# andres-fr/realtime-pose-estimation

Hardware: AMD Instinct MI355X
Metric: images/sec at 640x640 (HRNet-w48 fwd+decode) (higher is better)
Workload: dtype f16 (fp32 accumulate, fp32 BatchNorm; fp32 NCHW in/out); 1 GPU; configs[2]: batch=32 per GPU, 640x640, half-wrapper teacher forward + decode of 17 keypoint channels, weights W0 (seeded random); batch_per_gpu=32, people_per_batch_rank0=960

## Files before the change

### realtime-pose-estimation_amd/csrc/engine.hip

```cpp
#include <stdarg.h>

#include <chrono>
#include <mutex>
#include <map>
#include <tuple>
#include <vector>

#include "rtpe_common.h"

namespace rtpe {

static thread_local std::string g_err;

void set_error(const char* fmt, ...) {
  char buf[1024];
  va_list ap;
  va_start(ap, fmt);
  vsnprintf(buf, sizeof(buf), fmt, ap);
  va_end(ap);
  g_err = buf;
}

int hip_fail(hipError_t e, const char* what, const char* file, int line) {
  set_error("HIP error %d (%s) at %s:%d: %s", (int)e, hipGetErrorString(e), file, line, what);
// ... 9 lines not shown
  int n_geom;
  int fuse;
  int pair;
  int proj_head;
  int proj_op;
  int stem2;
  int s2g;
};

}

using namespace rtpe;

enum {
  kRouteNone = 0,
  kRouteTile, kRouteStream, kRouteDirect, kRouteConv64,
  kRouteHead,
  kRouteS2,
  kRouteS2Group,
  kRouteDeconvMerged, kRouteDeconv48,
  kRoutePairHead, kRoutePairTail, kRoutePairProj,
  kRouteBlock,
  kRouteStemFused, kRouteStemConv1, kRouteStemPlain,
  kRouteDoneBy
};
static_assert(kRouteTile == RTPE_ROUTE_TILE && kRouteHead == RTPE_ROUTE_HEAD && kRouteS2 == RTPE_ROUTE_S2 && kRouteS2Group == RTPE_ROUTE_S2_GROUP &&
              kRouteDeconvMerged == RTPE_ROUTE_DECONV_MERGED && kRoutePairHead == RTPE_ROUTE_PAIR_HEAD && kRoutePairTail == RTPE_ROUTE_PAIR_TAIL &&
              kRoutePairProj == RTPE_ROUTE_PAIR_PROJ && kRouteBlock == RTPE_ROUTE_BLOCK && kRouteStemFused == RTPE_ROUTE_STEM_FUSED &&
              kRouteStemConv1 == RTPE_ROUTE_STEM_CONV1 && kRouteStemPlain == RTPE_ROUTE_STEM_PLAIN && kRouteDoneBy == RTPE_ROUTE_DONE_BY,
              "rtpe_hip_trace.h names other route numbers");

static void trace_put(std::vector<int32_t>* tr, int kind, int a, int b, int c = 0, int d = 0) {
  const int32_t r[RTPE_TRACE_INTS] = {kind, a, b, c, d};
  tr->insert(tr->end(), r, r + RTPE_TRACE_INTS);
}

struct Route {
  int how, by;
  ConvTile tile[4];
};

struct rtpe_record {
  std::vector<hipEvent_t> ev;
  std::vector<Route> routes;
};

struct rtpe_hrnet {
// ... 1 lines not shown
  std::vector<OpState> ops;
  std::map<std::tuple<int, int, int>, std::vector<ConvTile>> tuned;
  std::map<int, rtpe_record> records;
  std::vector<rtpe_tensor_desc> tensors;
  std::vector<char> plane_ok;
  int n_slots;
  char* arena;
  size_t arena_bytes;
  int n_preds, n_refined;
  std::mutex lane_mu;
  hipStream_t lane_stream[4] = {nullptr, nullptr, nullptr, nullptr};
  std::vector<hipEvent_t> op_event;
  std::vector<char> needs_event;
  std::vector<std::vector<int>> wait_ops;
  hipEvent_t fork_event = nullptr;
  bool has_regions = false;
  std::vector<int32_t> trace;
  bool any_size = false;
};

static size_t align_up(size_t v, size_t a) { return (v + a - 1) / a * a; }

namespace rtpe {
static int g_options[kNumOptions] = {-1, -1, -1, -1, -1, -1, -1, -1, -1, -1, -1, -1};
static const char* const kOptionNames[kNumOptions] = {"block_ring", "block_pc", "direct_1x1", "lanes", "tile_dma", "pair_1x1", "fused_stem", "conv64", "head_direct", "deconv48", "conv48s2", "pair_proj"};
static const char* const kOptionEnv[kNumOptions] = {"RTPE_BLOCK_RING", "RTPE_BLOCK_PC", "RTPE_DIRECT_1X1", "RTPE_LANES", "RTPE_TILE_DMA", "RTPE_PAIR_1X1", "RTPE_FUSED_STEM", "RTPE_CONV64", "RTPE_HEAD_DIRECT", "RTPE_DECONV48", "RTPE_CONV48S2", "RTPE_PAIR_PROJ"};
static const int kOptionDefault[kNumOptions] = {0, 1, 1, 1, 1, 1, 1, 1, 1, 1, 1, 1};
int get_option(int key) {
  int v = __atomic_load_n(&g_options[key], __ATOMIC_RELAXED);
  if (v < 0) {
    v = kOptionEnv[key][0] ? env_int(kOptionEnv[key], kOptionDefault[key]) : kOptionDefault[key];
    __atomic_store_n(&g_options[key], v, __ATOMIC_RELAXED);
  }
  return v;
}
}

extern "C" int rtpe_set_option(const char* name, int32_t value) {
  RTPE_REQUIRE(name != nullptr && value >= 0, "set_option: bad argument");
  for (int k = 0; k < kNumOptions; ++k)
    if (kOptionNames[k][0] && strcmp(name, kOptionNames[k]) == 0) {
      __atomic_store_n(&g_options[k], (int)value, __ATOMIC_RELAXED);
      return RTPE_OK;
    }
  set_error("set_option: unknown option '%s'", name);
  return RTPE_E_INVALID;
}

extern "C" int rtpe_get_option(const char* name, int32_t* value) {
  RTPE_REQUIRE(name != nullptr && value != nullptr, "get_option: null argument");
  for (int k = 0; k < kNumOptions; ++k)
    if (kOptionNames[k][0] && strcmp(name, kOptionNames[k]) == 0) {
      *value = get_option(k);
      return RTPE_OK;
// ... 425 lines not shown

static std::vector<char> plane_tensors(const rtpe_hrnet* h, int N, int H, int W, const std::vector<ConvTile>* tuned, bool rag) {
  if (rag) return std::vector<char>(h->plane_ok.size(), 0);
  std::vector<char> plane = h->plane_ok;
  for (size_t i = 0; i < h->ops.size(); ++i) {
    const OpState& o = h->ops[i];
    const rtpe_op_desc& d = o.d;
    if (d.kind != RTPE_OP_CONV || o.n_geom != 1) continue;
    if (!(plane[d.in_t] || plane[d.out_t] || (d.res_t >= 0 && plane[d.res_t]))) continue;
    const rtpe_tensor_desc& ti = h->tensors[d.in_t];
    const ConvTile t = (tuned && (*tuned)[i * 4].nt) ? (*tuned)[i * 4]
                                                      : conv_make_tile(o.plan[0], N, extent(H, ti.ds_log2), extent(W, ti.ds_log2));
    if (t.kind != 2) {
      plane[d.in_t] = plane[d.out_t] = 0;
      if (d.res_t >= 0) plane[d.res_t] = 0;
    }
  }
  return plane;
}

struct RouteOpts {
  int fused_stem = get_option(kOptFusedStem), pair_1x1 = get_option(kOptPair1x1), pair_proj = get_option(kOptPairProj),
      conv64 = get_option(kOptConv64), head_direct = get_option(kOptHeadDirect), deconv48 = get_option(kOptDeconv48),
      conv48s2 = get_option(kOptConv48s2);
};

struct Fwd {
  const rtpe_hrnet* h;
  int N, H, W;
  char* base;
  void *preds, *refined;
  int out_dtype;
  std::vector<size_t> offs;
  size_t ws_need;
  const std::vector<ConvTile>* tuned = nullptr;
  std::vector<char> plane;
  bool rag;
  const int32_t* ext;
  const int32_t* level(int ds) const { return ext + (size_t)ds * 2 * N; }
  Fwd(const rtpe_hrnet* h_, int N_, int H_, int W_, void* ws, void* preds_, void* refined_, int out_dtype_, const int32_t* ext_ = nullptr)
      : h(h_), N(N_), H(H_), W(W_), base(reinterpret_cast<char*>(ws)), preds(preds_), refined(refined_), out_dtype(out_dtype_),
        rag(ragged(H_, W_) || ext_ != nullptr), ext(ext_) {
    slot_layout(h, N, H, W, &offs, &ws_need);
    auto it = h->tuned.find(std::make_tuple(N, H, W));
    if (it != h->tuned.end() && !rag) tuned = &it->second;
    plane = plane_tensors(h, N, H, W, tuned, rag);
  }
// ... 72 lines not shown
    a.ext_in = f.level(ti.ds_log2);
    a.ext_out = f.level(ti.ds_log2 + (d.stride == 2 ? 1 : 0));
  }
  return a;
}

static ConvArgs conv_op_args(const Fwd& f, size_t i, int k, const ConvTile& t) {
  ConvArgs a = conv_op_args(f, i, k);
  conv_fill_args(f.h->ops[i].geom[k], f.h->ops[i].plan[k], t, &a);
  return a;
}

static bool conv_direct_ok(const ConvArgs& a) {
  return a.x_bytes < 0x80000000ull && a.y != nullptr && a.y_nchw == nullptr && a.o_mul == 1;
}

static void conv_fix_tile(const RouteOpts& opt, const ConvPlan& p, const ConvArgs& a, bool plane_io, ConvTile* t) {
  const bool direct_ok = conv_direct_ok(a);
  if (t->kind == 4 && !direct_ok) *t = conv_make_tile(p, a.N, a.H_pos, a.W_pos, false);
  if (t->kind == 5 && !(direct_ok && a.res == nullptr && !plane_io && opt.conv64 != 0))
    *t = conv_make_tile(p, a.N, a.H_pos, a.W_pos, true, false);
}

static int conv_pick(const RouteOpts& opt, const ConvPlan& p, const ConvTile& t, const ConvArgs& a, bool plane_io) {
  if (opt.head_direct != 0 && conv_head_supports(p, a)) return kRouteHead;
  if (opt.conv48s2 != 0 && !plane_io && conv48s2_supports(p, a)) return kRouteS2;
  return t.kind == 2 ? kRouteStream : t.kind == 4 ? kRouteDirect : t.kind == 5 ? kRouteConv64 : kRouteTile;
}

static bool deconv_merges(const ConvPlan* p, const ConvTile& tile0) {
  static const int merge_deconv = env_int("RTPE_DECONV_MERGE", 1);
  bool merge = merge_deconv && tile0.kind == 0;
  for (int k = 1; k < 4 && merge; ++k)
    merge = p[k].mt == p[0].mt && p[k].cc == p[0].cc && p[k].kc == p[0].kc && p[k].n_cchunks == p[0].n_cchunks &&
            p[k].n_cb == p[0].n_cb && p[k].pstride == p[0].pstride && p[k].tapw == p[0].tapw;
  return merge;
}

static void deconv_merge_class(ConvArgs* merged, const ConvArgs& a, int k) {
  if (k == 0) { *merged = a; merged->n_cls = 4; }
  merged->w_c[k] = a.w;
  merged->lo_yc[k] = a.lo_y; merged->lo_xc[k] = a.lo_x;
  merged->oy_c[k] = a.oy_add; merged->ox_c[k] = a.ox_add;
}

static ConvArgs deconv_merged_args(const Fwd& f, size_t i, const ConvTile& tile0) {
  ConvArgs merged;
  for (int k = 0; k < 4; ++k) deconv_merge_class(&merged, conv_op_args(f, i, k, tile0), k);
  return merged;
}

static int deconv_pick(const RouteOpts& opt, const ConvPlan& p0, const ConvArgs& merged) {
  return opt.deconv48 != 0 && deconv48_supports(p0, merged) ? kRouteDeconv48 : kRouteDeconvMerged;
}

static int launch_conv(int how, const ConvPlan& p, const ConvTile& t, const ConvArgs& a, hipStream_t s) {
  switch (how) {
    case kRouteHead: return conv_head_launch(p, a, s);
    case kRouteS2: return conv48s2_launch(p, a, s);
    case kRouteDeconv48: return deconv48_launch(p, a, s);
    default: return conv_launch(p, t, a, s);
  }
}

static int route_ops(const Fwd& f, std::vector<Route>* routes, std::vector<ConvArgs>* args) {
  const rtpe_hrnet* h = f.h;
  const RouteOpts opt;
  routes->assign(h->ops.size(), Route());
  args->assign(h->ops.size(), ConvArgs());
  for (size_t i = 0; i < h->ops.size(); ++i) {
    Route& r = (*routes)[i];
    const OpState& o = h->ops[i];
    const rtpe_op_desc& d = o.d;
    auto absorb = [&](size_t j) { (*routes)[j].how = kRouteDoneBy; (*routes)[j].by = (int)i; };
    if (r.how == kRouteDoneBy) continue;
    if (d.kind == RTPE_OP_STEM) {
      const int fused = !f.rag && stem_fused_supports(f.H, f.W) ? opt.fused_stem : 0;
      r.how = fused == 1 && o.stem2 == 1 ? kRouteStemFused : fused == 2 && !(d.flags & RTPE_F_F32) ? kRouteStemConv1 : kRouteStemPlain;
      if (r.how == kRouteStemFused) absorb(i + 1);
      continue;
    }
    if (o.n_geom == 0) continue;
// ... 21 lines not shown
    if (o.s2g > 1 && opt.conv48s2 != 0) {
      bool ok = true;
      for (int m = 0; m < o.s2g && ok; ++m) {
        const OpState& om = h->ops[i + m];
        Route& rm = (*routes)[i + m];
        if (m > 0) rm.tile[0] = f.tile(i + m, 0, Hi / 2, Wi / 2);
        (*args)[i + m] = conv_op_args(f, i + m, 0, rm.tile[0]);
        ok = !f.plane[om.d.in_t] && !f.plane[om.d.out_t] && conv48s2_supports(om.plan[0], (*args)[i + m]);
      }
      if (ok) {
        r.how = kRouteS2Group;
        r.by = o.s2g;
        for (int m = 1; m < o.s2g; ++m) absorb(i + m);
        continue;
      }
    }
    const bool plane_io = f.plane[d.in_t] || (!(d.flags & RTPE_F_NO_NHWC) && f.plane[d.out_t]);
    ConvArgs& a = (*args)[i];
    a = conv_op_args(f, i, 0);
    for (int k = 0; k < o.n_geom; ++k) conv_fix_tile(opt, o.plan[k], k ? conv_op_args(f, i, k) : a, plane_io, &r.tile[k]);
    conv_fill_args(o.geom[0], o.plan[0], r.tile[0], &a);
    if (r.how == kRoutePairTail) continue;
    r.how = conv_pick(opt, o.plan[0], r.tile[0], a, plane_io);
    if (r.how == kRouteHead || r.how == kRouteS2 || opt.pair_1x1 == 0 || !conv_direct_ok(a)) continue;
    if (o.proj_head > 0 && opt.pair_proj != 0 && conv_direct_ok(conv_op_args(f, o.proj_head, 0))) {
      r.how = kRoutePairProj;
      r.by = o.proj_head + 1;
    } else if (o.pair == 1) {
      r.how = kRoutePairHead;
      r.by = (int)i + 1;
      (*routes)[i + 1].how = kRoutePairTail;
      (*routes)[i + 1].by = (int)i;
    }
  }
  for (size_t i = 0; i < h->ops.size(); ++i)
    RTPE_REQUIRE((*routes)[i].how != kRoutePairProj || (*routes)[h->ops[i].proj_head].how == kRoutePairHead,
                 "forward: op %d is no 1x1 pair head at this shape, its projection was folded", h->ops[i].proj_head);
  return RTPE_OK;
}

static void route_label(const rtpe_hrnet* h, const std::vector<Route>& routes, size_t i, int32_t* out8) {
  const Route& r = routes[i];
  const OpState& o = h->ops[i];
  const ConvTile& t = r.tile[0];
  const int by = r.how == kRouteDoneBy ? routes[r.by].how : kRouteNone;
  auto set = [&](int mt, int nt, int waves, int th, int tw, int cc, int n_cb, int v) {
    const int32_t l[8] = {mt, nt, waves, th, tw, cc, n_cb, v};
    memcpy(out8, l, sizeof(l));
  };
  memset(out8, 0, 8 * sizeof(int32_t));
  if (r.how == kRouteStemFused || by == kRouteStemFused) {
    set(4, 4, 8, 8, 16, 64, 1, by ? -600002 : -600001);
  } else if (r.how == kRouteBlock || by == kRouteBlock) {
    set(3, by ? 3 : 5, 4, 6, 32, 48, 1, by ? -900002 : -900001);
  } else if (r.how == kRouteS2 || r.how == kRouteS2Group || by == kRouteS2Group) {
    const int gw = o.d.cout == 48 ? 1 : o.d.cout == 96 ? 2 : 4;
    set(3, 2, 4, 8, 8, 48, o.d.cout / (48 * gw), by ? -200009 : r.how == kRouteS2Group ? -(200000 + r.by) : -200001);
  } else if (r.how == kRouteHead) {
    set(o.plan[0].mt, 2, 4, 1, 32, 48, 1, -400001);
  } else if (r.how == kRouteDeconv48) {
    set(3, 2, 4, 8, 16, 48, 1, -300001);
  } else if (r.how == kRoutePairProj) {
    set(0, 1, 8, 1, 16, 64, 1, -800003);
  } else if (r.how == kRoutePairHead || r.how == kRoutePairTail) {
    const bool head = r.how == kRoutePairHead;
    set(head ? 16 : 4, 1, 8, 1, 16, head ? 64 : 256, 1, head ? -800001 : -800002);
  } else if (o.n_geom > 0) {
    set(t.kind == 0 && t.mrun ? t.mrun : o.plan[0].mt, t.nt, t.waves, t.th, t.tw, o.plan[0].cc, o.plan[0].n_cb,
        t.kind == 2 ? -(t.grid + 100000 * t.n_bufs) : t.kind == 4 ? -(700000 + t.grid) : t.kind == 5 ? -(500000 + t.grid) : (int32_t)t.lds_bytes);
  }
}

static bool block_head(const std::vector<Route>& r, size_t i) { return i < r.size() && r[i].how == kRouteBlock; }
static bool block_tail(const std::vector<Route>& r, size_t i) { return i > 0 && block_head(r, i - 1); }

static bool op_has_event(const std::vector<Route>& r, size_t i) {
  return !block_tail(r, i) && !(block_head(r, i) && block_head(r, i + 2));
}

static int read_op_times(const std::vector<Route>& r, const std::vector<hipEvent_t>& ev, float* op_ms) {
// ... 219 lines not shown
  const Route& r = routes[i];
  switch (r.how) {
    case kRouteDoneBy: case kRoutePairHead: case kRoutePairProj:
      return RTPE_OK;
    case kRouteStemFused: case kRouteStemConv1:
      return stem_fused_launch(stem_fused_args(f, c, i, r.how == kRouteStemFused), s);
    case kRouteStemPlain:
      return stem_launch(stem_args(f, c, i), s);
    case kRouteBlock:
      return launch_block(f, i, s);
    case kRouteS2Group: {
      const ConvPlan* plans[3];
      for (int m = 0; m < r.by; ++m) plans[m] = &h->ops[i + m].plan[0];
      return conv48s2_launch_group(plans, &args[i], r.by, s);
    }
    case kRoutePairTail: {
      const OpState& oh = h->ops[r.by];
      const bool proj = oh.proj_op >= 0 && routes[oh.proj_op].how == kRoutePairProj;
      return conv_pair_launch(oh.plan[0], args[r.by], o.plan[0], args[i], s, proj ? &h->ops[oh.proj_op].plan[0] : nullptr,
                              proj ? &args[oh.proj_op] : nullptr);
    }
    case kRouteDeconvMerged: case kRouteDeconv48:
      return launch_conv(r.how, o.plan[0], r.tile[0], args[i], s);
    case kRouteTile: case kRouteStream: case kRouteDirect: case kRouteConv64: case kRouteHead: case kRouteS2: {
      int rc = launch_conv(r.how, o.plan[0], r.tile[0], args[i], s);
      for (int k = 1; k < o.n_geom && rc == RTPE_OK; ++k)
        rc = launch_conv(r.how, o.plan[k], r.tile[k], conv_op_args(f, i, k, r.tile[k]), s);
      return rc;
    }
    default:
      break;
  }
  switch (o.d.kind) {
    case RTPE_OP_CAST: case RTPE_OP_AUX_PACK: case RTPE_OP_RESIZE: case RTPE_OP_GATE_MUL:
      return launch_f32_op(f, c, i, s);
    case RTPE_OP_AVGPOOL: case RTPE_OP_SE: case RTPE_OP_CAM_COMBINE: case RTPE_OP_SIGMOID_ADD:
      return (o.d.flags & RTPE_F_F32) ? launch_student_op<float>(f, c, i, s) : launch_student_op<_Float16>(f, c, i, s);
    default:
      return launch_fuse(f, i, s);
  }
}

class Lanes {
 public:
  Lanes(rtpe_hrnet* h, const FwdCall& c, const std::vector<Route>& routes, std::vector<int32_t>* trace)
      : h_(h), routes_(routes), main_(c.stream), tr_(trace) {
    if (h->has_regions && c.op_ms == nullptr && c.rec == nullptr && !(c.flags & RTPE_FWD_NO_LANES)) {
// ... 434 lines not shown
  a.alpha = reinterpret_cast<const float*>(dev + wb); a.beta = a.alpha + p.cout_pad;
  a.res = reinterpret_cast<const _Float16*>(res); a.res_ld = cout;
  a.y = reinterpret_cast<_Float16*>(y); a.out_ld = cout; a.cout_store = cout;
  a.N = N; a.H_in = H; a.W_in = W;
  a.H_full = a.H_pos = H / stride; a.W_full = a.W_pos = W / stride; a.o_mul = 1;
  a.relu = (flags & RTPE_F_RELU) ? 1 : 0;
  a.round_conv = (flags & RTPE_F_ROUND_CONV) ? 1 : 0;
  const RouteOpts opt;
  ConvTile tile = conv_make_tile(p, N, a.H_pos, a.W_pos);
  conv_fix_tile(opt, p, a, false, &tile);
  static const int probe_plane = RTPE_DIAG_ENV_INT("RTPE_PROBE_PLANE", 0);
  if (probe_plane && tile.kind == 2 && cin % 48 == 0 && cout % 48 == 0 && stride == 1) {
    a.in_ld = 48; a.in_cs = (long long)N * H * W * 48;
    a.out_ld = 48; a.out_cs = (long long)N * H * W * 48;
    if (res != nullptr) { a.res_ld = 48; a.res_cs = (long long)N * H * W * 48; }
  }
  conv_fill_args(g, p, tile, &a);
#ifdef RTPE_CONV_STAMPS
  unsigned long long* dbg = nullptr;
  hipMalloc(reinterpret_cast<void**>(&dbg), 128);
  hipMemset(dbg, 0, 128);
  a.dbg = dbg;
#endif
  int rc = launch_conv(conv_pick(opt, p, tile, a, false), p, tile, a, s);
  hipError_t es2 = hipStreamSynchronize(s);
#ifdef RTPE_CONV_STAMPS
  unsigned long long hd[16];
  hipMemcpy(hd, dbg, 128, hipMemcpyDeviceToHost);
  hipFree(dbg);
  if (tile.kind == 2 && hd[5] && (hd[11] = hd[11] ? hd[11] : hd[5] / tile.waves)) {
    const unsigned long long nw = (unsigned long long)tile.grid * tile.waves, units = hd[5] / p.n_cchunks;
    fprintf(stderr, "stream conv %dx%d nt%d w%d nb%d nw%d grid %d | per MFMA wave: total %llu cycles, %llu units | per stage: waitM %llu half0 %llu "
            "waitH %llu half1 %llu | per unit: E-wait %llu bn+transpose %llu res-wait %llu rows+add+store %llu load_res %llu | weight loader/stage: wait %llu issue %llu | "
            "tile loaders/stage: wait %llu issue %llu\n",
            tile.th, tile.tw, tile.nt, tile.waves, tile.n_bufs, tile.n_wslots, tile.grid, hd[15] / nw, units / nw, hd[0] / hd[5], hd[1] / hd[5],
            hd[2] / hd[5], hd[3] / hd[5], hd[12] / units, hd[13] / units, hd[4] / units, hd[14] / units, hd[10] / units, hd[6] / hd[11],
            hd[7] / hd[11], hd[8] / hd[11], hd[9] / hd[11]);
  }
  else if (hd[5])
    fprintf(stderr, "conv stamps (kind %d): n %llu | per wave(-unit) cycles: setup %llu stage/wait1 %llu kloop %llu epilogue %llu total/wait2 %llu\n",
            tile.kind, hd[5], hd[0] / hd[5], hd[1] / hd[5], hd[2] / hd[5], hd[3] / hd[5], hd[4] / hd[5]);
  if (hd[10] && tile.kind != 2)
    fprintf(stderr, "   loader per stage: vmcnt-wait %llu barrier1 %llu issue %llu barriersE+2 %llu (stages %llu)\n",
            hd[6] / hd[10], hd[7] / hd[10], hd[8] / hd[10], hd[9] / hd[10], hd[10]);
#endif
  hipFree(dev);
  if (rc != RTPE_OK) return rc;
  if (es2 != hipSuccess) return hip_fail(es2, "hipStreamSynchronize", __FILE__, __LINE__);
  return RTPE_OK;
}

extern "C" int rtpe_basicblock_nhwc(const void* x, int32_t N, int32_t H, int32_t W, const void* w1_host,
                                    const float* alpha1, const float* beta1, const void* w2_host, const float* alpha2,
                                    const float* beta2, void* y, void* stream) {
  RTPE_REQUIRE(x && w1_host && w2_host && alpha1 && beta1 && alpha2 && beta2 && y, "basicblock_nhwc: null argument");
  RTPE_REQUIRE(conv_block_supports(48, 48, H, W), "basicblock_nhwc: H=%d W=%d unsupported", H, W);
  hipStream_t s = reinterpret_cast<hipStream_t>(stream);
  ConvGeom g{48, 48, 3, 1, -1, 2, 1};
  ConvPlan p = conv_make_plan(g);
  const size_t wb = align_up(p.packed_bytes, 256), abb = align_up(2 * 48 * sizeof(float), 256);
// ... 346 lines not shown
```

### realtime-pose-estimation_amd/csrc/rtpe_common.h

```cpp
#pragma once
#include <hip/hip_runtime.h>
#include <hip/hip_fp16.h>
#include <stdint.h>
#include <stdio.h>
#include <stdlib.h>
#include <string.h>
#include <string>
#include <vector>

#include "rtpe_hip.h"

namespace rtpe {

void set_error(const char* fmt, ...);
int hip_fail(hipError_t e, const char* what, const char* file, int line);

#define RTPE_HIP_CHECK(expr)                                               \
  do {                                                                     \
    hipError_t _e = (expr);                                                \
    if (_e != hipSuccess) return ::rtpe::hip_fail(_e, #expr, __FILE__, __LINE__); \
  } while (0)

#define RTPE_REQUIRE(cond, ...)                 \
  do {                                          \
    if (!(cond)) {                              \
      ::rtpe::set_error(__VA_ARGS__);           \
      return RTPE_E_INVALID;                    \
    }                                           \
  } while (0)

inline int env_int(const char* name, int dflt) {
  const char* v = getenv(name);
  return v ? atoi(v) : dflt;
}
#ifdef RTPE_DIAG
#define RTPE_DIAG_ENV_INT(name, dflt) ::rtpe::env_int(name, dflt)
#else
#define RTPE_DIAG_ENV_INT(name, dflt) (dflt)
#endif

enum { kOptBlockRing = 0, kOptBlockPC = 1, kOptDirect1x1 = 2, kOptLanes = 3, kOptTileDma = 4, kOptPair1x1 = 5, kOptFusedStem = 6, kOptConv64 = 7, kOptHeadDirect = 8, kOptDeconv48 = 9, kOptConv48s2 = 10, kOptPairProj = 11, kNumOptions = 12 };
int get_option(int key);

inline bool first_use_on_device(unsigned long long* mask) {
  int dev = 0;
  if (hipGetDevice(&dev) != hipSuccess || dev < 0 || dev > 63) return true;
  const unsigned long long bit = 1ull << dev;
  const unsigned long long old = __atomic_fetch_or(mask, bit, __ATOMIC_RELAXED);
  return !(old & bit);
}

struct DeviceGuard {
  int prev = -1;
  bool switched = false;
  hipError_t err = hipSuccess;
  explicit DeviceGuard(int device) {
    err = hipGetDevice(&prev);
    if (err == hipSuccess && prev != device) {
      err = hipSetDevice(device);
      switched = err == hipSuccess;
    }
  }
  ~DeviceGuard() {
    if (switched) (void)hipSetDevice(prev);
// ... 132 lines not shown
void conv_enum_tiles(const ConvPlan& p, int N, int H_pos, int W_pos, std::vector<ConvTile>* out);
void conv_pack_weights(const ConvGeom& g, const ConvPlan& p, const void* w, void* packed);
void conv_fill_args(const ConvGeom& g, const ConvPlan& p, const ConvTile& t, ConvArgs* a);
int conv_launch(const ConvPlan& p, const ConvTile& t, const ConvArgs& a, hipStream_t s);
bool conv_stream_supports(const ConvPlan& p);
size_t conv_stream_lds(const ConvPlan& p, int buf_bytes, int n_bufs, int n_wslots);
int conv_stream_launch(const ConvPlan& p, const ConvTile& t, const ConvArgs& a, hipStream_t s);
bool conv_pair_supports(int cin1, int cout1, int cout2);
int conv_pair_launch(const ConvPlan& p1, const ConvArgs& c1, const ConvPlan& p2, const ConvArgs& c2, hipStream_t s,
                     const ConvPlan* pd = nullptr, const ConvArgs* cd = nullptr);
int conv_direct_mb(const ConvPlan& p);
bool conv64_supports(const ConvPlan& p);
size_t conv64_lds();
int conv64_grid(int N, int H_pos, int W_pos);
int conv64_launch(const ConvPlan& p, const ConvTile& t, const ConvArgs& a, hipStream_t s);
int conv_direct_launch(const ConvPlan& p, const ConvArgs& a, hipStream_t s);
bool conv_head_supports(const ConvPlan& p, const ConvArgs& a);
int conv_head_launch(const ConvPlan& p, const ConvArgs& a, hipStream_t s);
bool deconv48_supports(const ConvPlan& p, const ConvArgs& merged);
int deconv48_launch(const ConvPlan& p, const ConvArgs& merged, hipStream_t s);
bool conv48s2_supports(const ConvPlan& p, const ConvArgs& a);
int conv48s2_launch(const ConvPlan& p, const ConvArgs& a, hipStream_t s);
int conv48s2_launch_group(const ConvPlan* const* plans, const ConvArgs* layers, int n, hipStream_t s);
bool conv_block_supports(int cin, int cout, int H, int W);
int conv_block_launch(const _Float16* x, int in_ld, size_t x_bytes, _Float16* y, int out_ld, const _Float16* w1,
                      const float* ab1, const _Float16* w2, const float* ab2, int N, int H, int W, hipStream_t s);

struct FuseArgs {
  const _Float16* term[4];
  int term_ld[4], term_up[4];
  int n_terms;
  _Float16* y;
  int out_ld, C;
  int N, H, W;
  int f32;
  int relu;
  int nearest;
  int term_h[4], term_w[4];
  const int* ext_out;
  const int* ext_term[4];
};
int fuse_launch(const FuseArgs& a, hipStream_t s);
bool fuse_nearest_supports(int N, int H, int W, int C, int f32);

struct StemArgs {
  const void* x;
// ... 54 lines not shown
```

Baseline: 2480 images/sec.

## Add warp-specialized stride-2 3x3 conv kernel for wide-channel transition layers

Adds a new stride-2 3x3 convolution kernel with dedicated loader waves. One wave streams weights and two waves stream input tiles into LDS through double-buffered buffer-to-LDS loads, while four MFMA waves compute and run a fused BN/ReLU epilogue. It is routed by default for the 96->192/384 and 192->384 downsampling layers and replaces the generic stream or tile conv path for them. It adds another specialized kernel and more barrier synchronization in exchange for better overlap of memory and compute on these layers.

```diff
diff --git a/include/rtpe_hip_s2c.h b/include/rtpe_hip_s2c.h
--- /dev/null
+++ b/include/rtpe_hip_s2c.h
@@ -0,0 +1,20 @@
+#ifndef RTPE_HIP_S2C_H
+#define RTPE_HIP_S2C_H
+
+#include <stdint.h>
+
+#ifdef __cplusplus
+extern "C" {
+#endif
+
+int rtpe_conv_s2c_probe(int32_t cin, int32_t cout, int32_t ksize, int32_t stride, int32_t N, int32_t H, int32_t W,
+                        int32_t in_ld, int32_t plane, int32_t with_res, int32_t small_grid, int32_t* out10);
+
+int rtpe_conv_s2c_layer(const void* x, int32_t N, int32_t H, int32_t W, int32_t in_ld, int32_t in_coff, int32_t cin,
+                        const void* w_host, const float* alpha_host, const float* beta_host, int32_t cout, int32_t flags,
+                        void* y, void* stream, int32_t kernel);
+
+#ifdef __cplusplus
+}
+#endif
+#endif
diff --git a/realtime-pose-estimation_amd/csrc/conv_s2c.hip b/realtime-pose-estimation_amd/csrc/conv_s2c.hip
--- /dev/null
+++ b/realtime-pose-estimation_amd/csrc/conv_s2c.hip
@@ -0,0 +1,450 @@
+#include "conv_stream_dev.h"
+#include "conv_s2c_host.h"
+
+namespace rtpe {
+
+namespace {
+constexpr int kMulWaves = 4;
+constexpr int kThreads = (kMulWaves + kLoaders) * 64;
+constexpr int kRowB = kS2cRowBytes;
+constexpr int kHH = 17, kHW = 17, kNEven = 9;
+constexpr int kRowSlots = kHW * kSlots;
+constexpr int kTileStep = 4 * kRowB;
+static_assert(kRowB >= kHW * kPStride && kS2cBufBytes >= kHH * kRowB, "tile image");
+
+struct S2cArgs {
+  const _Float16* x;
+  const _Float16* w;
+  const float* alpha;
+  const float* beta;
+  _Float16* y;
+  unsigned x_bytes, y_bytes, w_bytes;
+  int N, H_in, W_in, in_ld, H_out, W_out, out_ld, cout_store, relu;
+  int ncc, n_cb, tiles_x, tiles_y, ablate;
+  FastDiv div_tiles_x, div_tiles_xy;
+  unsigned long long* dbg;
+};
+}
+
+template <int MT, bool ROUND>
+__global__ void __launch_bounds__(kThreads) conv_s2c_kernel(const S2cArgs a) {
+  constexpr int NT = MT == 6 ? 2 : 1;
+  constexpr int WSLOT = MT * kKH * 1024;
+  extern __shared__ __attribute__((aligned(16))) char smem[];
+  char* const wring = smem;
+  char* const tiles = smem + 2 * WSLOT;
+  const int tid = threadIdx.x, lane = tid & 63;
+  const int wv = __builtin_amdgcn_readfirstlane(tid >> 6);
+
+  Units um;
+  um.init(a.N * a.tiles_x * a.tiles_y, a.n_cb);
+  const uint32_t tiles_xy = (uint32_t)(a.tiles_x * a.tiles_y);
+  const int ncc = a.ncc;
+  const int sh = __builtin_ctz((unsigned)ncc);
+  const int S = um.count << sh;
+  if (S == 0) return;
+
+  if (wv == kMulWaves) {
+    __amdgpu_buffer_rsrc_t rsrc = __builtin_amdgcn_make_buffer_rsrc(const_cast<_Float16*>(a.w), 0, (int)a.w_bytes, 0x00020000);
+    const int voff = lane * 16;
+    auto issue = [&](int q) {
+      const int s = q >> 1, h = q & 1;
+      int tile, cb;
+      um.get(s >> sh, &tile, &cb);
+      const int cci = s & (ncc - 1);
+      const int src = ((cb * ncc + cci) * kKC + h * kKH) * MT * 1024;
+      char* dst = wring + h * WSLOT;
+#pragma unroll
+      for (int p = 0; p < MT * kKH; ++p)
+        __builtin_amdgcn_raw_ptr_buffer_load_lds(rsrc, (lds_ptr_t)(dst + p * 1024), 16, voff, src + p * 1024, 0, 0);
+    };
+#ifdef RTPE_CONV_STAMPS
+    unsigned long long w0, w1, w2, w3, w4, wwait = 0, wissue = 0;
+#endif
+    issue(0);
+    for (int s = 0; s < S; ++s) {
+      SSTAMP(w0);
+      asm volatile("s_waitcnt vmcnt(0)" ::: "memory");
+      SSTAMP(w1);
+      RTPE_SBARRIER();
+      SSTAMP(w2);
+      issue(2 * s + 1);
+      SSTAMP(w3);
+      asm volatile("s_waitcnt vmcnt(0)" ::: "memory");
+      SSTAMP(w4);
+      RTPE_SBARRIER();
+      if (s + 1 < S) issue(2 * s + 2);
+      if ((s & (ncc - 1)) == ncc - 1) RTPE_SBARRIER();
+#ifdef RTPE_CONV_STAMPS
+      wwait += (w1 - w0) + (w4 - w3); wissue += w3 - w2;
+#endif
+    }
+    asm volatile("s_waitcnt vmcnt(0)" ::: "memory");
+#ifdef RTPE_CONV_STAMPS
+    if (a.dbg != nullptr && lane == 0) { atomicAdd(&a.dbg[6], wwait); atomicAdd(&a.dbg[7], wissue); atomicAdd(&a.dbg[11], (unsigned long long)S); }
+#endif
+    return;
+  }
+
+  if (wv > kMulWaves) {
+    const int jl = wv - kMulWaves - 1;
+    __amdgpu_buffer_rsrc_t rsrc = __builtin_amdgcn_make_buffer_rsrc(const_cast<_Float16*>(a.x), 0, (int)a.x_bytes, 0x00020000);
+    struct TileReq {
+      uint32_t voff[2];
+      int soff0, soff_row;
+      int row_lo, row_hi;
+      char* buf;
+    };
+    auto prepare = [&](int s, TileReq& q) {
+      int tile, cb;
+      um.get(s >> sh, &tile, &cb);
+      const int chunk = s & (ncc - 1);
+      uint32_t t = (uint32_t)tile;
+      const uint32_t n = fdiv(t, a.div_tiles_xy);
+      t -= n * tiles_xy;
+      const uint32_t tyi = fdiv(t, a.div_tiles_x);
+      const uint32_t txi = t - tyi * a.tiles_x;
+      const int iy0 = (int)tyi * (2 * kS2cTile) - 1, ix0 = (int)txi * (2 * kS2cTile) - 1;
+#pragma unroll
+      for (int k = 0; k < 2; ++k) {
+        const int qq = k * 64 + lane;
+        const int lc = qq / kSlots, sl = qq - lc * kSlots;
+        const int col = lc < kNEven ? 2 * lc : 2 * (lc - kNEven) + 1;
+        const int ix = ix0 + col;
+        const bool ok = qq < kRowSlots && (unsigned)ix < (unsigned)a.W_in;
+        q.voff[k] = ok ? (uint32_t)(ix * a.in_ld + sl * 8) * 2u : 0x80000000u;
+      }
+      q.buf = tiles + (s & 1) * kS2cBufBytes;
+      q.soff_row = a.W_in * a.in_ld * 2;
+      q.soff0 = (((int)n * a.H_in + iy0) * a.W_in * a.in_ld + chunk * kCC) * 2;
+      q.row_lo = iy0 < 0 ? -iy0 : 0;
+      q.row_hi = a.H_in - iy0;
+    };
+    auto fire = [&](const TileReq& q, int r0, int r1) {
+      for (int r = r0; r < r1; ++r) {
+        const bool row_ok = r >= q.row_lo && r < q.row_hi;
+        const int soff = row_ok ? q.soff0 + r * q.soff_row : 0;
+        char* dst = q.buf + r * kRowB;
+        __builtin_amdgcn_raw_ptr_buffer_load_lds(rsrc, (lds_ptr_t)dst, 16, (int)(row_ok ? q.voff[0] : 0x80000000u), soff, 0, 0);
+        if (lane < kRowSlots - 64)
+          __builtin_amdgcn_raw_ptr_buffer_load_lds(rsrc, (lds_ptr_t)(dst + 1024), 16, (int)(row_ok ? q.voff[1] : 0x80000000u), soff, 0, 0);
+      }
+    };
+    const int ra = jl == 0 ? 0 : (kHH + 1) / 2, rb = jl == 0 ? (kHH + 1) / 2 : kHH;
+#ifdef RTPE_CONV_STAMPS
+    unsigned long long t0, t1, t2, t3, twait = 0, tissue = 0;
+#endif
+    {
+      TileReq q;
+      prepare(0, q);
+      if (!(a.ablate & 4)) fire(q, ra, rb);
+    }
+    for (int s = 0; s < S; ++s) {
+      SSTAMP(t0);
+      const bool more = s + 1 < S;
+      TileReq q;
+      prepare(more ? s + 1 : S - 1, q);
+      asm volatile("s_waitcnt vmcnt(0)" ::: "memory");
+      SSTAMP(t1);
+      RTPE_SBARRIER();
+      SSTAMP(t2);
+      if (more && !(a.ablate & 4)) fire(q, ra, rb);
+      SSTAMP(t3);
+      RTPE_SBARRIER();
+      if ((s & (ncc - 1)) == ncc - 1) RTPE_SBARRIER();
+#ifdef RTPE_CONV_STAMPS
+      twait += t1 - t0; tissue += t3 - t2;
+#endif
+    }
+    asm volatile("s_waitcnt vmcnt(0)" ::: "memory");
+#ifdef RTPE_CONV_STAMPS
+    if (a.dbg != nullptr && lane == 0) { atomicAdd(&a.dbg[8], twait); atomicAdd(&a.dbg[9], tissue); }
+#endif
+    return;
+  }
+
+  const int r = lane & 15, g = lane >> 4;
+  const int ch = MT == 6 ? (wv & 1) : 0;
+  const int pt0 = MT == 6 ? (wv >> 1) * 2 : wv;
+  int toff[kKC];
+#pragma unroll
+  for (int kk = 0; kk < kKC; ++kk) {
+    int k = kk * 32 + g * 8;
+    if (k >= 9 * kCC) k -= 9 * kCC;
+    const int tap = k / kCC, c = k - tap * kCC;
+    const int ty = tap / 3, tx = tap - ty * 3;
+    const int cs = tx == 0 ? 0 : tx == 1 ? kNEven : 1;
+    toff[kk] = ty * kRowB + cs * kPStride + c * 2;
+  }
+  const int lane_off = pt0 * kTileStep + 2 * (r >> 3) * kRowB + (r & 7) * kPStride;
+
+  constexpr int ROWB = 3 * 32 + 16;
+  constexpr int CH = 6;
+  constexpr int NIT = (NT * 16 * CH + 63) / 64;
+  int tile0, cb0;
+  um.get(0, &tile0, &cb0);
+  const int chan0 = (cb0 * MT + ch * 3) * 16;
+  float4v al[3], be[3];
+#pragma unroll
+  for (int m = 0; m < 3; ++m) {
+    const int c4 = chan0 + m * 16 + g * 4;
+    al[m] = *reinterpret_cast<const float4v*>(a.alpha + c4);
+    be[m] = *reinterpret_cast<const float4v*>(a.beta + c4);
+  }
+#pragma unroll
+  for (int m = 0; m < 3; ++m) asm volatile("" ::"v"(al[m]), "v"(be[m]));
+  __amdgpu_buffer_rsrc_t ysrc = __builtin_amdgcn_make_buffer_rsrc(a.y, 0, (int)a.y_bytes, 0x00020000);
+  int eoff[NIT], orel[NIT], oyx[NIT];
+#pragma unroll
+  for (int it = 0; it < NIT; ++it) {
+    const int c = it * 64 + lane;
+    const int pw = c / CH, slot = c - pw * CH;
+    const int T = pt0 + (pw >> 4), rr = pw & 15;
+    const int oy = 2 * T + (rr >> 3), ox = rr & 7;
+    const bool valid = c < NT * 16 * CH && chan0 + slot * 8 < a.cout_store;
+    eoff[it] = c < NT * 16 * CH ? pw * ROWB + slot * 16 : 0;
+    orel[it] = ((oy * a.W_out + ox) * a.out_ld + chan0 + slot * 8) * 2;
+    oyx[it] = valid ? (oy | (ox << 8)) : 0x4000;
+  }
+
+  float4v acc[3][NT];
+  auto half_stage = [&](const char* wslot, const char* tb, auto hsel) {
+    constexpr int H = decltype(hsel)::value;
+    const char* wl = wslot + ch * 3 * 1024 + lane * 16;
+    half8 af[2][3], bf[2][NT];
+#pragma unroll
+    for (int m = 0; m < 3; ++m) af[0][m] = *reinterpret_cast<const half8*>(wl + m * 1024);
+#pragma unroll
+    for (int nt = 0; nt < NT; ++nt) bf[0][nt] = *reinterpret_cast<const half8*>(tb + nt * kTileStep + toff[H * kKH]);
+#pragma unroll
+    for (int kk = 0; kk < kKH; ++kk) {
+      const int cur = kk & 1, nxt = cur ^ 1;
+      if (kk + 1 < kKH) {
+#pragma unroll
+        for (int m = 0; m < 3; ++m) af[nxt][m] = *reinterpret_cast<const half8*>(wl + ((kk + 1) * MT + m) * 1024);
+#pragma unroll
+        for (int nt = 0; nt < NT; ++nt) bf[nxt][nt] = *reinterpret_cast<const half8*>(tb + nt * kTileStep + toff[H * kKH + kk + 1]);
+      }
+#pragma unroll
+      for (int m = 0; m < 3; ++m)
+#pragma unroll
+        for (int nt = 0; nt < NT; ++nt)
+          acc[m][nt] = __builtin_amdgcn_mfma_f32_16x16x32_f16(af[cur][m], bf[cur][nt], acc[m][nt], 0, 0, 0);
+      if (kk + 1 < kKH) {
+#pragma unroll
+        for (int i = 0; i < (3 + NT + 2) / 3; ++i) {
+          __builtin_amdgcn_sched_group_barrier(0x008, 1, 0);
+          __builtin_amdgcn_sched_group_barrier(0x002, 3, 0);
+          __builtin_amdgcn_sched_group_barrier(0x100, 3, 0);
+        }
+      }
+      __builtin_amdgcn_sched_barrier(0);
+    }
+  };
+
+#ifdef RTPE_CONV_STAMPS
+  unsigned long long st[16] = {0};
+  const unsigned long long k_begin = __builtin_readcyclecounter();
+#endif
+  int s = 0;
+  const int n_units = um.count;
+  for (int u = 0; u < n_units; ++u) {
+#ifdef RTPE_CONV_STAMPS
+    unsigned long long m0, m1, m2, m3, m4;
+#endif
+    int tile, cb;
+    um.get(u, &tile, &cb);
+    uint32_t t = (uint32_t)tile;
+    const uint32_t n = fdiv(t, a.div_tiles_xy);
+    t -= n * tiles_xy;
+    const uint32_t tyi = fdiv(t, a.div_tiles_x);
+    const int py0 = (int)tyi * kS2cTile, px0 = (int)(t - tyi * a.tiles_x) * kS2cTile;
+#pragma unroll
+    for (int m = 0; m < 3; ++m)
+#pragma unroll
+      for (int nt = 0; nt < NT; ++nt) acc[m][nt] = float4v{0.f, 0.f, 0.f, 0.f};
+    char* tilebuf = nullptr;
+    for (int cci = 0; cci < ncc; ++cci, ++s) {
+      tilebuf = tiles + (s & 1) * kS2cBufBytes;
+      SSTAMP(m0);
+      RTPE_SBARRIER();
+      SSTAMP(m1);
+      if (!(a.ablate & 1)) half_stage(wring, tilebuf + lane_off, std::integral_constant<int, 0>());
+      SSTAMP(m2);
+      RTPE_SBARRIER();
+      SSTAMP(m3);
+      if (!(a.ablate & 1)) half_stage(wring + WSLOT, tilebuf + lane_off, std::integral_constant<int, 1>());
+      SSTAMP(m4);
+#ifdef RTPE_CONV_STAMPS
+      st[0] += m1 - m0; st[1] += m3 - m2; st[2] += (m2 - m1) + (m4 - m3); st[5] += 1;
+#endif
+    }
+    asm volatile("s_waitcnt lgkmcnt(0)" ::: "memory");
+    SSTAMP(m0);
+    RTPE_SBARRIER();
+    SSTAMP(m1);
+    char* obuf = tilebuf + wv * (NT * 16 * ROWB);
+#pragma unroll
+    for (int nt = 0; nt < NT; ++nt) {
+#pragma unroll
+      for (int m = 0; m < 3; ++m) {
+        const float4v v = acc[m][nt];
+        half4 o;
+        if (ROUND) {
+          o = bn_round(v, al[m], be[m]);
+        } else {
+          float2v lo{v[0], v[1]}, hi{v[2], v[3]};
+          lo = __builtin_elementwise_fma(lo, float2v{al[m][0], al[m][1]}, float2v{be[m][0], be[m][1]});
+          hi = __builtin_elementwise_fma(hi, float2v{al[m][2], al[m][3]}, float2v{be[m][2], be[m][3]});
+          const half2v olo = __builtin_convertvector(lo, half2v), ohi = __builtin_convertvector(hi, half2v);
+          o = half4{olo[0], olo[1], ohi[0], ohi[1]};
+        }
+        *reinterpret_cast<half4*>(obuf + (nt * 16 + r) * ROWB + m * 32 + g * 8) = o;
+      }
+    }
+    half8 ov[NIT];
+#pragma unroll
+    for (int it = 0; it < NIT; ++it) ov[it] = *reinterpret_cast<const half8*>(obuf + eoff[it]);
+    const int pix0 = ((int)n * a.H_out + py0) * a.W_out + px0;
+    const int ly = a.H_out - py0, lx = a.W_out - px0;
+#pragma unroll
+    for (int it = 0; it < NIT; ++it) {
+      if (a.relu) {
+        short8 b = __builtin_bit_cast(short8, ov[it]);
+        b = b & ~(b >> 15);
+        ov[it] = __builtin_bit_cast(half8, b);
+      }
+      const bool ok = (oyx[it] & 0x40ff) < ly && ((oyx[it] >> 8) & 0x3f) < lx && !(a.ablate & 2);
+      const uint32_t voff = ok ? (uint32_t)(pix0 * a.out_ld * 2 + orel[it]) : 0x80000000u;
+      __builtin_amdgcn_raw_buffer_store_b128(__builtin_bit_cast(u32x4, ov[it]), ysrc, (int)voff, 0, 0);
+    }
+    asm volatile("s_waitcnt lgkmcnt(0)" ::: "memory");
+#ifdef RTPE_CONV_STAMPS
+    { unsigned long long m5; SSTAMP(m5); st[3] += m5 - m1; st[4] += m1 - m0; }
+#endif
+  }
+#ifdef RTPE_CONV_STAMPS
+  if (a.dbg != nullptr && lane == 0) {
+    st[15] = __builtin_readcyclecounter() - k_begin;
+    const int slots[] = {0, 1, 2, 3, 4, 5, 15};
+    for (int i : slots) atomicAdd(&a.dbg[i], st[i]);
+    atomicAdd(&a.dbg[12], 1ull);
+  }
+#endif
+}
+
+bool conv_s2c_supports(const ConvPlan& p, const ConvArgs& a) { return s2c_supports(p, a); }
+
+template <int MT>
+static int conv_s2c_launch_mt(const S2cArgs& a, const S2cLayout& l, bool round_conv, hipStream_t s) {
+  static unsigned long long attr_mask = 0;
+  if (first_use_on_device(&attr_mask)) {
+    RTPE_HIP_CHECK(hipFuncSetAttribute(reinterpret_cast<const void*>(conv_s2c_kernel<MT, false>), hipFuncAttributeMaxDynamicSharedMemorySize, 160 * 1024));
+    RTPE_HIP_CHECK(hipFuncSetAttribute(reinterpret_cast<const void*>(conv_s2c_kernel<MT, true>), hipFuncAttributeMaxDynamicSharedMemorySize, 160 * 1024));
+  }
+  if (round_conv) hipLaunchKernelGGL((conv_s2c_kernel<MT, true>), dim3((unsigned)l.grid), dim3(kThreads), (size_t)l.lds_bytes, s, a);
+  else hipLaunchKernelGGL((conv_s2c_kernel<MT, false>), dim3((unsigned)l.grid), dim3(kThreads), (size_t)l.lds_bytes, s, a);
+  RTPE_HIP_CHECK(hipGetLastError());
+  return RTPE_OK;
+}
+
+static int conv_s2c_launch_grid(const ConvPlan& p, const ConvArgs& c, hipStream_t s, bool small_grid) {
+  RTPE_REQUIRE(conv_s2c_supports(p, c), "conv_s2c: unsupported layer");
+  const S2cLayout l = s2c_layout(p.mt, p.n_cb, c.N, c.H_full, c.W_full, small_grid);
+  RTPE_REQUIRE(l.lds_bytes <= 160 * 1024 && l.units < (1l << 20) && l.grid % 8 == 0 && (l.grid / 8) % p.n_cb == 0,
+               "conv_s2c: layout (%d B of LDS, %ld units, grid %d)", l.lds_bytes, l.units, l.grid);
+  S2cArgs a;
+  memset(&a, 0, sizeof(a));
+  a.x = c.x; a.w = c.w; a.alpha = c.alpha; a.beta = c.beta; a.y = c.y;
+  a.x_bytes = (unsigned)c.x_bytes;
+  a.y_bytes = (unsigned)s2c_out_bytes(c);
+  a.w_bytes = (unsigned)p.packed_bytes;
+  a.N = c.N; a.H_in = c.H_in; a.W_in = c.W_in; a.in_ld = c.in_ld; a.H_out = c.H_full; a.W_out = c.W_full; a.out_ld = c.out_ld;
+  a.cout_store = c.cout_store; a.relu = c.relu;
+  a.ncc = p.n_cchunks; a.n_cb = p.n_cb; a.tiles_x = l.tiles_x; a.tiles_y = l.tiles_y; a.ablate = c.ablate;
+  a.div_tiles_x = make_fastdiv((uint32_t)l.tiles_x);
+  a.div_tiles_xy = make_fastdiv((uint32_t)(l.tiles_x * l.tiles_y));
+  a.dbg = c.dbg;
+  return p.mt == 6 ? conv_s2c_launch_mt<6>(a, l, c.round_conv != 0, s) : conv_s2c_launch_mt<3>(a, l, c.round_conv != 0, s);
+}
+
+int conv_s2c_launch(const ConvPlan& p, const ConvArgs& c, hipStream_t s) {
+  return conv_s2c_launch_grid(p, c, s, get_option(kOptConvS2c) == 2);
+}
+
+}
+
+extern "C" int rtpe_conv_s2c_probe(int32_t cin, int32_t cout, int32_t ksize, int32_t stride, int32_t N, int32_t H, int32_t W,
+                                   int32_t in_ld, int32_t plane, int32_t with_res, int32_t small_grid, int32_t* out10) {
+  using namespace rtpe;
+  RTPE_REQUIRE(out10 != nullptr && cin > 0 && cout > 0 && N > 0 && H > 0 && W > 0 && (stride == 1 || stride == 2) &&
+               (ksize == 1 || ksize == 3), "conv_s2c_probe: bad argument");
+  ConvGeom g{cin, cout, ksize, stride, -1, 2, 1};
+  const ConvPlan p = conv_make_plan(g);
+  ConvArgs a;
+  memset(&a, 0, sizeof(a));
+  static _Float16 dummy[8] __attribute__((aligned(16)));
+  a.x = dummy; a.y = dummy; a.w = dummy;
+  a.res = with_res ? dummy : nullptr;
+  a.in_ld = in_ld ? in_ld : cin;
+  a.x_bytes = (size_t)N * H * W * a.in_ld * 2;
+  if (plane) { a.in_ld = 48; a.in_cs = (long long)N * H * W * 48; }
+  a.out_ld = cout; a.cout_store = cout; a.res_ld = cout;
+  a.N = N; a.H_in = H; a.W_in = W;
+  a.H_full = a.H_pos = (H + stride - 1) / stride; a.W_full = a.W_pos = (W + stride - 1) / stride; a.o_mul = 1;
+  ConvTile t = conv_make_tile(p, N, a.H_pos, a.W_pos, false, false, false);
+  conv_fill_args(g, p, t, &a);
+  const S2cLayout l = s2c_layout(p.mt, p.n_cb, N, a.H_full, a.W_full, small_grid != 0);
+  const int32_t v[10] = {conv_s2c_supports(p, a) ? 1 : 0, l.wslot_bytes, l.ring_bytes, l.buf_bytes, l.n_bufs, l.lds_bytes,
+                         l.tiles_x, l.tiles_y, (int32_t)l.units, l.grid};
+  memcpy(out10, v, sizeof(v));
+  return RTPE_OK;
+}
+
+extern "C" int rtpe_conv_s2c_layer(const void* x, int32_t N, int32_t H, int32_t W, int32_t in_ld, int32_t in_coff, int32_t cin,
+                                   const void* w_host, const float* alpha_host, const float* beta_host, int32_t cout,
+                                   int32_t flags, void* y, void* stream, int32_t kernel) {
+  using namespace rtpe;
+  RTPE_REQUIRE(x && w_host && alpha_host && beta_host && y && N > 0 && H > 0 && W > 0 && cin % 8 == 0 && cout % 8 == 0 &&
+               in_coff >= 0 && in_coff % 8 == 0 && in_coff + cin <= in_ld && kernel >= 0 && kernel <= 2,
+               "conv_s2c_layer: bad argument");
+  hipStream_t s = reinterpret_cast<hipStream_t>(stream);
+  ConvGeom g{cin, cout, 3, 2, -1, 2, 1};
+  const ConvPlan p = conv_make_plan(g);
+  std::vector<char> packed(p.packed_bytes);
+  conv_pack_weights(g, p, w_host, packed.data());
+  std::vector<float> ab(2 * p.cout_pad, 0.f);
+  for (int c = 0; c < cout; ++c) { ab[c] = alpha_host[c]; ab[p.cout_pad + c] = beta_host[c]; }
+  char* dev = nullptr;
+  const size_t wb = (p.packed_bytes + 255) / 256 * 256;
+  RTPE_HIP_CHECK(hipMalloc(reinterpret_cast<void**>(&dev), wb + ab.size() * 4));
+  hipError_t e = hipMemcpy(dev, packed.data(), p.packed_bytes, hipMemcpyHostToDevice);
+  if (e == hipSuccess) e = hipMemcpy(dev + wb, ab.data(), ab.size() * 4, hipMemcpyHostToDevice);
+  if (e != hipSuccess) { hipFree(dev); return hip_fail(e, "hipMemcpy", __FILE__, __LINE__); }
+  ConvArgs a;
+  memset(&a, 0, sizeof(a));
+  a.x = reinterpret_cast<const _Float16*>(x) + in_coff; a.in_ld = in_ld;
+  a.x_bytes = ((size_t)N * H * W * in_ld - (size_t)in_coff) * 2;
+  a.w = reinterpret_cast<const _Float16*>(dev);
+  a.alpha = reinterpret_cast<const float*>(dev + wb); a.beta = a.alpha + p.cout_pad;
+  a.y = reinterpret_cast<_Float16*>(y); a.out_ld = cout; a.cout_store = cout;
+  a.N = N; a.H_in = H; a.W_in = W;
+  a.H_full = a.H_pos = (H + 1) / 2; a.W_full = a.W_pos = (W + 1) / 2; a.o_mul = 1;
+  a.relu = (flags & RTPE_F_RELU) ? 1 : 0;
+  a.round_conv = (flags & RTPE_F_ROUND_CONV) ? 1 : 0;
+  const ConvTile t = conv_make_tile(p, N, a.H_pos, a.W_pos, false, false, false);
+  conv_fill_args(g, p, t, &a);
+  int rc;
+  if (kernel == 0) {
+    rc = conv_launch(p, t, a, s);
+  } else if (!conv_s2c_supports(p, a)) {
+    set_error("conv_s2c_layer: the kernel does not take this layer");
+    rc = RTPE_E_INVALID;
+  } else {
+    rc = conv_s2c_launch_grid(p, a, s, kernel == 2);
+  }
+  const hipError_t es = hipStreamSynchronize(s);
+  hipFree(dev);
+  if (rc == RTPE_OK && es != hipSuccess) return hip_fail(es, "hipStreamSynchronize", __FILE__, __LINE__);
+  return rc;
+}
diff --git a/realtime-pose-estimation_amd/csrc/conv_s2c_host.h b/realtime-pose-estimation_amd/csrc/conv_s2c_host.h
--- /dev/null
+++ b/realtime-pose-estimation_amd/csrc/conv_s2c_host.h
@@ -0,0 +1,55 @@
+#pragma once
+#include "rtpe_common.h"
+
+namespace rtpe {
+
+constexpr int kS2cTile = 8;
+constexpr int kS2cRowBytes = 1664;
+constexpr int kS2cBufBytes = (17 * kS2cRowBytes + 255) / 256 * 256;
+constexpr int kS2cBufs = 2;
+
+struct S2cLayout {
+  int wslot_bytes;
+  int ring_bytes;
+  int buf_bytes, n_bufs;
+  int lds_bytes;
+  int tiles_x, tiles_y;
+  long units;
+  int grid;
+};
+
+inline S2cLayout s2c_layout(int mt, int n_cb, int N, int H_out, int W_out, bool small_grid) {
+  S2cLayout l;
+  l.wslot_bytes = mt * 7 * 1024;
+  l.ring_bytes = 2 * l.wslot_bytes;
+  l.buf_bytes = kS2cBufBytes;
+  l.n_bufs = kS2cBufs;
+  l.lds_bytes = l.ring_bytes + l.n_bufs * l.buf_bytes;
+  l.tiles_x = (W_out + kS2cTile - 1) / kS2cTile;
+  l.tiles_y = (H_out + kS2cTile - 1) / kS2cTile;
+  const long tiles = (long)N * l.tiles_x * l.tiles_y;
+  l.units = tiles * n_cb;
+  long G = small_grid ? 1 : 32;
+  const long need = (tiles + 7) / 8 * n_cb;
+  if (G > need) G = need;
+  G = (G + n_cb - 1) / n_cb * n_cb;
+  l.grid = (int)(8 * G);
+  return l;
+}
+
+inline size_t s2c_out_bytes(const ConvArgs& a) { return (size_t)a.N * a.H_full * a.W_full * a.out_ld * 2; }
+
+inline bool s2c_supports(const ConvPlan& p, const ConvArgs& a) {
+  if (!(p.esize == 2 && p.dil == 1 && p.tapw == 3 && p.in_mul == 2 && p.cc == 48 && p.kc == 14 && p.pstride == 96 &&
+        (p.cin == 96 || p.cin == 192) && p.n_cchunks * 48 == p.cin && (p.mt == 3 || p.mt == 6) && p.cout % 48 == 0 &&
+        p.cout_pad == p.cout && p.n_cb >= 1 && p.n_cb <= 32))
+    return false;
+  return a.n_cls == 0 && a.mixed == 0 && a.o_mul == 1 && a.res == nullptr && a.y != nullptr && a.y_nchw == nullptr &&
+         a.in_cs == 48 && a.out_cs == p.mt * 16 && a.in_ld >= p.cin && a.in_ld % 8 == 0 && a.out_ld >= p.cout &&
+         a.out_ld % 8 == 0 && a.cout_store % 8 == 0 && a.cout_store <= p.cout && a.cout_store > 0 &&
+         ((uintptr_t)a.x & 15) == 0 && ((uintptr_t)a.y & 15) == 0 && a.x_bytes > 0 && a.x_bytes < 0x80000000ull &&
+         s2c_out_bytes(a) < 0x80000000ull && a.H_pos == a.H_full && a.W_pos == a.W_full && a.H_pos == (a.H_in + 1) / 2 &&
+         a.W_pos == (a.W_in + 1) / 2 && a.lo_y == -1 && a.lo_x == -1;
+}
+
+}
diff --git a/realtime-pose-estimation_amd/csrc/engine.hip b/realtime-pose-estimation_amd/csrc/engine.hip
--- a/realtime-pose-estimation_amd/csrc/engine.hip
+++ b/realtime-pose-estimation_amd/csrc/engine.hip
@@ -55,7 +55,8 @@
   kRoutePairHead, kRoutePairTail, kRoutePairProj,
   kRouteBlock,
   kRouteStemFused, kRouteStemConv1, kRouteStemPlain,
-  kRouteDoneBy
+  kRouteDoneBy,
+  kRouteS2C
 };
 static_assert(kRouteTile == RTPE_ROUTE_TILE && kRouteHead == RTPE_ROUTE_HEAD && kRouteS2 == RTPE_ROUTE_S2 && kRouteS2Group == RTPE_ROUTE_S2_GROUP &&
               kRouteDeconvMerged == RTPE_ROUTE_DECONV_MERGED && kRoutePairHead == RTPE_ROUTE_PAIR_HEAD && kRoutePairTail == RTPE_ROUTE_PAIR_TAIL &&
@@ -103,14 +104,15 @@
 static size_t align_up(size_t v, size_t a) { return (v + a - 1) / a * a; }
 
 namespace rtpe {
-static int g_options[kNumOptions] = {-1, -1, -1, -1, -1, -1, -1, -1, -1, -1, -1, -1};
-static const char* const kOptionNames[kNumOptions] = {"block_ring", "block_pc", "direct_1x1", "lanes", "tile_dma", "pair_1x1", "fused_stem", "conv64", "head_direct", "deconv48", "conv48s2", "pair_proj"};
-static const char* const kOptionEnv[kNumOptions] = {"RTPE_BLOCK_RING", "RTPE_BLOCK_PC", "RTPE_DIRECT_1X1", "RTPE_LANES", "RTPE_TILE_DMA", "RTPE_PAIR_1X1", "RTPE_FUSED_STEM", "RTPE_CONV64", "RTPE_HEAD_DIRECT", "RTPE_DECONV48", "RTPE_CONV48S2", "RTPE_PAIR_PROJ"};
-static const int kOptionDefault[kNumOptions] = {0, 1, 1, 1, 1, 1, 1, 1, 1, 1, 1, 1};
+static int g_options[kNumOptions] = {-1, -1, -1, -1, -1, -1, -1, -1, -1, -1, -1, -1, -1};
+static const char* const kOptionNames[kNumOptions] = {"block_ring", "block_pc", "direct_1x1", "lanes", "tile_dma", "pair_1x1", "fused_stem", "conv64", "head_direct", "deconv48", "conv48s2", "pair_proj", "conv_s2c"};
+static const char* const kOptionEnv[kNumOptions] = {"RTPE_BLOCK_RING", "RTPE_BLOCK_PC", "RTPE_DIRECT_1X1", "RTPE_LANES", "RTPE_TILE_DMA", "RTPE_PAIR_1X1", "RTPE_FUSED_STEM", "RTPE_CONV64", "RTPE_HEAD_DIRECT", "RTPE_DECONV48", "RTPE_CONV48S2", "RTPE_PAIR_PROJ", "RTPE_CONV_S2C"};
+static const int kOptionDefault[kNumOptions] = {0, 1, 1, 1, 1, 1, 1, 1, 1, 1, 1, 1, 1};
 int get_option(int key) {
   int v = __atomic_load_n(&g_options[key], __ATOMIC_RELAXED);
   if (v < 0) {
     v = kOptionEnv[key][0] ? env_int(kOptionEnv[key], kOptionDefault[key]) : kOptionDefault[key];
+    if (key == kOptConvS2c && getenv(kOptionEnv[key]) == nullptr && !(env_int("RTPE_CONV_STREAM", 1) & 1)) v = 0;
     __atomic_store_n(&g_options[key], v, __ATOMIC_RELAXED);
   }
   return v;
@@ -582,7 +584,7 @@
 struct RouteOpts {
   int fused_stem = get_option(kOptFusedStem), pair_1x1 = get_option(kOptPair1x1), pair_proj = get_option(kOptPairProj),
       conv64 = get_option(kOptConv64), head_direct = get_option(kOptHeadDirect), deconv48 = get_option(kOptDeconv48),
-      conv48s2 = get_option(kOptConv48s2);
+      conv48s2 = get_option(kOptConv48s2), conv_s2c = get_option(kOptConvS2c);
 };
 
 struct Fwd {
@@ -701,9 +703,15 @@
     *t = conv_make_tile(p, a.N, a.H_pos, a.W_pos, true, false);
 }
 
+static bool conv_s2c_routed(const ConvPlan& p) {
+  if (get_option(kOptConvS2c) >= 2) return true;
+  return (p.cin == 96 && (p.cout == 192 || p.cout == 384)) || (p.cin == 192 && p.cout == 384);
+}
+
 static int conv_pick(const RouteOpts& opt, const ConvPlan& p, const ConvTile& t, const ConvArgs& a, bool plane_io) {
   if (opt.head_direct != 0 && conv_head_supports(p, a)) return kRouteHead;
   if (opt.conv48s2 != 0 && !plane_io && conv48s2_supports(p, a)) return kRouteS2;
+  if (opt.conv_s2c != 0 && !plane_io && conv_s2c_routed(p) && conv_s2c_supports(p, a)) return kRouteS2C;
   return t.kind == 2 ? kRouteStream : t.kind == 4 ? kRouteDirect : t.kind == 5 ? kRouteConv64 : kRouteTile;
 }
 
@@ -737,6 +745,7 @@
   switch (how) {
     case kRouteHead: return conv_head_launch(p, a, s);
     case kRouteS2: return conv48s2_launch(p, a, s);
+    case kRouteS2C: return conv_s2c_launch(p, a, s);
     case kRouteDeconv48: return deconv48_launch(p, a, s);
     default: return conv_launch(p, t, a, s);
   }
@@ -804,7 +813,7 @@
     conv_fill_args(o.geom[0], o.plan[0], r.tile[0], &a);
     if (r.how == kRoutePairTail) continue;
     r.how = conv_pick(opt, o.plan[0], r.tile[0], a, plane_io);
-    if (r.how == kRouteHead || r.how == kRouteS2 || opt.pair_1x1 == 0 || !conv_direct_ok(a)) continue;
+    if (r.how == kRouteHead || r.how == kRouteS2 || r.how == kRouteS2C || opt.pair_1x1 == 0 || !conv_direct_ok(a)) continue;
     if (o.proj_head > 0 && opt.pair_proj != 0 && conv_direct_ok(conv_op_args(f, o.proj_head, 0))) {
       r.how = kRoutePairProj;
       r.by = o.proj_head + 1;
@@ -838,6 +847,9 @@
   } else if (r.how == kRouteS2 || r.how == kRouteS2Group || by == kRouteS2Group) {
     const int gw = o.d.cout == 48 ? 1 : o.d.cout == 96 ? 2 : 4;
     set(3, 2, 4, 8, 8, 48, o.d.cout / (48 * gw), by ? -200009 : r.how == kRouteS2Group ? -(200000 + r.by) : -200001);
+  } else if (r.how == kRouteS2C) {
+    const int mt = o.plan[0].mt;
+    set(mt == 6 ? -3 : 3, mt == 6 ? 2 : 1, 4, 8, 8, 48, o.plan[0].n_cb, -1100001);
   } else if (r.how == kRouteHead) {
     set(o.plan[0].mt, 2, 4, 1, 32, 48, 1, -400001);
   } else if (r.how == kRouteDeconv48) {
@@ -1103,7 +1115,7 @@
     }
     case kRouteDeconvMerged: case kRouteDeconv48:
       return launch_conv(r.how, o.plan[0], r.tile[0], args[i], s);
-    case kRouteTile: case kRouteStream: case kRouteDirect: case kRouteConv64: case kRouteHead: case kRouteS2: {
+    case kRouteTile: case kRouteStream: case kRouteDirect: case kRouteConv64: case kRouteHead: case kRouteS2: case kRouteS2C: {
       int rc = launch_conv(r.how, o.plan[0], r.tile[0], args[i], s);
       for (int k = 1; k < o.n_geom && rc == RTPE_OK; ++k)
         rc = launch_conv(r.how, o.plan[k], r.tile[k], conv_op_args(f, i, k, r.tile[k]), s);
@@ -1584,7 +1596,8 @@
   hipMemset(dbg, 0, 128);
   a.dbg = dbg;
 #endif
-  int rc = launch_conv(conv_pick(opt, p, tile, a, false), p, tile, a, s);
+  const int how = conv_pick(opt, p, tile, a, false);
+  int rc = launch_conv(how, p, tile, a, s);
   hipError_t es2 = hipStreamSynchronize(s);
 #ifdef RTPE_CONV_STAMPS
   unsigned long long hd[16];
@@ -1598,6 +1611,13 @@
             tile.th, tile.tw, tile.nt, tile.waves, tile.n_bufs, tile.n_wslots, tile.grid, hd[15] / nw, units / nw, hd[0] / hd[5], hd[1] / hd[5],
             hd[2] / hd[5], hd[3] / hd[5], hd[12] / units, hd[13] / units, hd[4] / units, hd[14] / units, hd[10] / units, hd[6] / hd[11],
             hd[7] / hd[11], hd[8] / hd[11], hd[9] / hd[11]);
+  }
+  else if (how == kRouteS2C && hd[5] && hd[11]) {
+    const unsigned long long units = hd[5] / p.n_cchunks;
+    fprintf(stderr, "conv_s2c stamps: per multiplier wave: total %llu cycles | per stage: waitM %llu waitH %llu k loops %llu | per unit: "
+            "E-wait %llu epilogue %llu | weight loader/stage: wait %llu issue %llu | tile loaders/stage: wait %llu issue %llu\n",
+            hd[15] / (hd[12] ? hd[12] : 1), hd[0] / hd[5], hd[1] / hd[5], hd[2] / hd[5], hd[4] / units, hd[3] / units,
+            hd[6] / hd[11], hd[7] / hd[11], hd[8] / (2 * hd[11]), hd[9] / (2 * hd[11]));
   }
   else if (hd[5])
     fprintf(stderr, "conv stamps (kind %d): n %llu | per wave(-unit) cycles: setup %llu stage/wait1 %llu kloop %llu epilogue %llu total/wait2 %llu\n",
diff --git a/realtime-pose-estimation_amd/csrc/rtpe_common.h b/realtime-pose-estimation_amd/csrc/rtpe_common.h
--- a/realtime-pose-estimation_amd/csrc/rtpe_common.h
+++ b/realtime-pose-estimation_amd/csrc/rtpe_common.h
@@ -39,7 +39,7 @@
 #define RTPE_DIAG_ENV_INT(name, dflt) (dflt)
 #endif
 
-enum { kOptBlockRing = 0, kOptBlockPC = 1, kOptDirect1x1 = 2, kOptLanes = 3, kOptTileDma = 4, kOptPair1x1 = 5, kOptFusedStem = 6, kOptConv64 = 7, kOptHeadDirect = 8, kOptDeconv48 = 9, kOptConv48s2 = 10, kOptPairProj = 11, kNumOptions = 12 };
+enum { kOptBlockRing = 0, kOptBlockPC = 1, kOptDirect1x1 = 2, kOptLanes = 3, kOptTileDma = 4, kOptPair1x1 = 5, kOptFusedStem = 6, kOptConv64 = 7, kOptHeadDirect = 8, kOptDeconv48 = 9, kOptConv48s2 = 10, kOptPairProj = 11, kOptConvS2c = 12, kNumOptions = 13 };
 int get_option(int key);
 
 inline bool first_use_on_device(unsigned long long* mask) {
@@ -218,6 +218,8 @@
 bool conv48s2_supports(const ConvPlan& p, const ConvArgs& a);
 int conv48s2_launch(const ConvPlan& p, const ConvArgs& a, hipStream_t s);
 int conv48s2_launch_group(const ConvPlan* const* plans, const ConvArgs* layers, int n, hipStream_t s);
+bool conv_s2c_supports(const ConvPlan& p, const ConvArgs& a);
+int conv_s2c_launch(const ConvPlan& p, const ConvArgs& a, hipStream_t s);
 bool conv_block_supports(int cin, int cout, int H, int W);
 int conv_block_launch(const _Float16* x, int in_ld, size_t x_bytes, _Float16* y, int out_ld, const _Float16* w1,
                       const float* ab1, const _Float16* w2, const float* ab2, int N, int H, int W, hipStream_t s);
```

Result: no change. 2457 images/sec (-0.9%).
